# GuyTevet/motion-diffusion-model

Measured on NVIDIA H100. Metric: motions/sec, higher is better.
Workload: dtype fp16 operands / fp32 accumulate (in/out projections hi-lo split)

## Files before the change

motion-diffusion-model_b200/csrc/attention_tc.cuh:

```cuda
#pragma once
#include <cuda_fp16.h>

#include "epilogues.cuh"
#include "ptx.cuh"

namespace b200 {

constexpr int ATC_THREADS = 128;
constexpr int ATC_QROWS = 64;
constexpr int ATC_TILES_PER_CTA = 4;
constexpr int ATC_DH = 128;
constexpr int ATC_MAX_KEYS = 256;

__host__ __device__ constexpr int atc_keys(int S) { return S <= 64 ? 64 : S <= 208 ? 208 : 256; }

struct AttnTcSmem {
  static __host__ __device__ int total(int keys) { return 1024 + 4 * keys * 128; }
};

template <int KEYS, bool WIDE>
__global__ void __launch_bounds__(ATC_THREADS, 2)
attention_tc_kernel(const __grid_constant__ CUtensorMap map_kv, const __half* __restrict__ qkv, __half* __restrict__ out,
                    const int* __restrict__ kvlen, int S, int d, float scale_log2) {
  constexpr int ATOM = KEYS * 128;
  constexpr int NS = KEYS / 2;
  constexpr int NB = KEYS / 16;
  extern __shared__ uint8_t smem_raw[];
  __shared__ uint64_t bar_k, bar_v;
  uint8_t* sK = reinterpret_cast<uint8_t*>((reinterpret_cast<uintptr_t>(smem_raw) + 1023) & ~uintptr_t(1023));
  uint8_t* sV = sK + 2 * ATOM;
  const int warp = threadIdx.x >> 5, lane = threadIdx.x & 31;
  const int h = blockIdx.x, smp = blockIdx.y;
  const int ld = 3 * d;
  const __half* base = qkv + static_cast<size_t>(smp) * S * ld;

  pdl_launch_dependents();
  if (threadIdx.x == 0) {
    tma_prefetch_desc(&map_kv);
    mbar_init(&bar_k, 1);
    mbar_init(&bar_v, 1);
    fence_barrier_init();
  }
  __syncthreads();
  pdl_wait();
  if (threadIdx.x == 0) {
    mbar_expect_tx(&bar_k, 2 * ATOM);
    for (int a = 0; a < 2; ++a) tma_load_3d(sK + a * ATOM, &map_kv, &bar_k, d + h * ATC_DH + 64 * a, 0, smp);
    mbar_expect_tx(&bar_v, 2 * ATOM);
    for (int a = 0; a < 2; ++a) tma_load_3d(sV + a * ATOM, &map_kv, &bar_v, 2 * d + h * ATC_DH + 64 * a, 0, smp);
  }

  const int kvl = min(kvlen[smp], S);
  const int nblk = max(1, (kvl + 15) >> 4);
  const int g = lane >> 2, t = lane & 3;
  const uint64_t desc_k = wgmma_desc_k_sw128(smem_u32(sK));
  const uint64_t desc_v = wgmma_desc_mn_sw128(smem_u32(sV), ATOM);
  const int ntiles = (S + ATC_QROWS - 1) / ATC_QROWS;
  const int ldo = (WIDE ? 2 : 1) * d;

  uint32_t qa[8][4];
  auto load_q = [&](int tile) {
    const int ra = tile * ATC_QROWS + warp * 16 + g, rb = ra + 8;
    const bool va = ra < S, vb = rb < S;
    const uint32_t* pa = reinterpret_cast<const uint32_t*>(base + static_cast<size_t>(va ? ra : 0) * ld + h * ATC_DH);
    const uint32_t* pb = reinterpret_cast<const uint32_t*>(base + static_cast<size_t>(vb ? rb : 0) * ld + h * ATC_DH);
#pragma unroll
    for (int ks = 0; ks < 8; ++ks) {
      qa[ks][0] = va ? pa[8 * ks + t] : 0u;
      qa[ks][1] = vb ? pb[8 * ks + t] : 0u;
      qa[ks][2] = va ? pa[8 * ks + 4 + t] : 0u;
      qa[ks][3] = vb ? pb[8 * ks + 4 + t] : 0u;
    }
  };
  if (static_cast<int>(blockIdx.z) < ntiles) load_q(blockIdx.z);
#pragma unroll 1
  for (int tile = blockIdx.z; tile < ntiles; tile += gridDim.z) {
    const int ra = tile * ATC_QROWS + warp * 16 + g, rb = ra + 8;
    const bool va = ra < S, vb = rb < S;
    float s[NS];
    mbar_wait(&bar_k, 0);
    wgmma_fence();
#pragma unroll
    for (int ks = 0; ks < 8; ++ks)
      WgmmaRA<KEYS, 0>::mma(s, qa[ks], desc_k + (((ks >> 2) * ATOM + (ks & 3) * 32) >> 4), ks != 0);
    wgmma_commit();
    wgmma_wait<0>();
    wgmma_fence_acc(s);
    float mxa = -INFINITY, mxb = -INFINITY;
#pragma unroll
    for (int j = 0; j < NS / 4; ++j)
#pragma unroll
      for (int i = 0; i < 2; ++i) {
        if (8 * j + 2 * t + i < kvl) {
          mxa = fmaxf(mxa, s[4 * j + i]);
          mxb = fmaxf(mxb, s[4 * j + 2 + i]);
        }
      }
#pragma unroll
    for (int o = 1; o < 4; o <<= 1) {
      mxa = fmaxf(mxa, __shfl_xor_sync(0xffffffffu, mxa, o));
      mxb = fmaxf(mxb, __shfl_xor_sync(0xffffffffu, mxb, o));
    }
    const float offa = (mxa == -INFINITY) ? 0.f : mxa * scale_log2;
    const float offb = (mxb == -INFINITY) ? 0.f : mxb * scale_log2;
    auto ex2 = [](float x) {
      float y;
      asm("ex2.approx.ftz.f32 %0, %1;" : "=f"(y) : "f"(x));
      return y;
    };
    uint32_t p[NB][4];
    float suma = 0.f, sumb = 0.f;
#pragma unroll
    for (int j = 0; j < NS / 4; ++j) {
      const int key = 8 * j + 2 * t;
      const float p0 = key < kvl ? ex2(fmaf(s[4 * j], scale_log2, -offa)) : 0.f;
      const float p1 = key + 1 < kvl ? ex2(fmaf(s[4 * j + 1], scale_log2, -offa)) : 0.f;
      const float p2 = key < kvl ? ex2(fmaf(s[4 * j + 2], scale_log2, -offb)) : 0.f;
      const float p3 = key + 1 < kvl ? ex2(fmaf(s[4 * j + 3], scale_log2, -offb)) : 0.f;
      suma += p0 + p1;
      sumb += p2 + p3;
      p[j >> 1][2 * (j & 1)] = pack_half2(p0, p1);
      p[j >> 1][2 * (j & 1) + 1] = pack_half2(p2, p3);
    }
#pragma unroll
    for (int off = 1; off < 4; off <<= 1) {
      suma += __shfl_xor_sync(0xffffffffu, suma, off);
      sumb += __shfl_xor_sync(0xffffffffu, sumb, off);
    }
    const float inva = suma > 0.f ? 1.f / suma : 0.f;
    const float invb = sumb > 0.f ? 1.f / sumb : 0.f;
    float o[64];
    mbar_wait(&bar_v, 0);
    wgmma_fence();
#pragma unroll
    for (int kk = 0; kk < NB; ++kk)
      if (kk < nblk) WgmmaRA<128, 1>::mma(o, p[kk], desc_v + ((kk * 16 * 128) >> 4), kk != 0);
    wgmma_commit();
    if (tile + static_cast<int>(gridDim.z) < ntiles) load_q(tile + gridDim.z);
    wgmma_wait<0>();
    wgmma_fence_acc(o);
    __half* oa = out + (static_cast<size_t>(smp) * S + (va ? ra : 0)) * ldo + h * ATC_DH + 2 * t;
    __half* ob = out + (static_cast<size_t>(smp) * S + (vb ? rb : 0)) * ldo + h * ATC_DH + 2 * t;
#pragma unroll
    for (int j = 0; j < 16; ++j) {
      const float x0 = o[4 * j] * inva, x1 = o[4 * j + 1] * inva, x2 = o[4 * j + 2] * invb, x3 = o[4 * j + 3] * invb;
      const __half2 ha = __floats2half2_rn(x0, x1), hb = __floats2half2_rn(x2, x3);
      if (va) *reinterpret_cast<__half2*>(oa + 8 * j) = ha;
      if (vb) *reinterpret_cast<__half2*>(ob + 8 * j) = hb;
      if (WIDE) {
        const float2 fa = __half22float2(ha), fb = __half22float2(hb);
        if (va) *reinterpret_cast<__half2*>(oa + d + 8 * j) = __floats2half2_rn(x0 - fa.x, x1 - fa.y);
        if (vb) *reinterpret_cast<__half2*>(ob + d + 8 * j) = __floats2half2_rn(x2 - fb.x, x3 - fb.y);
      }
    }
  }
}

}
```

motion-diffusion-model_b200/csrc/engine.cu:

```cuda
#include <cuda.h>
#include <cuda_fp16.h>
#include <cuda_runtime.h>

#include <algorithm>
#include <cmath>
#include <cstdarg>
#include <cstdio>
#include <cstring>
#include <initializer_list>
#include <map>
#include <string>
#include <vector>

#include "../../include/b200mdm.h"
#include "attention_tc.cuh"
#include "epilogues.cuh"
#include "gemm.cuh"
#include "gemm_ln.cuh"
#include "gemm_pingpong.cuh"
#include "chunk_frame.cuh"
#include "joint_guidance.cuh"
#include "compose.cuh"
#include "postprocess.cuh"
#include "kernels.cuh"
// ... 108 lines not shown
  bool operator==(const GraphKey& o) const {
    return mode == o.mode && B == o.B && T == o.T && flags == o.flags && order == o.order && pred == o.pred &&
           imask == o.imask && iweight == o.iweight && imotion == o.imotion && target_g == o.target_g && hs == o.hs &&
           guide == o.guide && chars == o.chars && groups == o.groups && slots == o.slots;
  }
};

struct Workspace {
  int B = 0, T = 0, S = 0, halves = 1, Bp = 0, M = 0, MB = 0;
  int groups = 0;
  float* mp_x0 = nullptr;
  __half *xin16 = nullptr, *hres = nullptr, *qkv16 = nullptr, *att16 = nullptr, *ffn16 = nullptr, *g16 = nullptr;
  float *tok0 = nullptr, *condproj = nullptr, *proj = nullptr, *scale = nullptr, *x_work = nullptr, *eps_buf = nullptr;
  int *kvlen = nullptr, *tvec = nullptr, *action = nullptr;
  CUtensorMap m_xin, m_h16, m_att, m_ffn, m_g16;
  CUtensorMap m_qkv_st, m_ffn_st;
  CUtensorMap m_qkv_kv;
  CUtensorMap m_res_c, m_res_u;
  CUtensorMap m_hres;
  float* pe_bias = nullptr;
  bool cond_set = false;
  int Mt = 0;
  float *encperm = nullptr, *memtok = nullptr, *memproj = nullptr;
  __half *mem16 = nullptr, *qc16 = nullptr, *kvc16 = nullptr;
  unsigned char* memmask = nullptr;
  CUtensorMap m_mem, m_qc_st, m_kvc_st;
  bool prefix_set = false;
  float *cross_mb = nullptr, *cross_u = nullptr, *cross_b = nullptr, *cross_c = nullptr;
  float *tgt_valid = nullptr, *tgt_g = nullptr;
  bool target_set = false;
  int* hs_desc = nullptr;
  bool hs_set = false;
  float* jg_x0 = nullptr;
  float *plms_ring = nullptr, *plms_mid = nullptr, *plms_pred = nullptr;
  int plms_done = -1, plms_order = 0;
  float* dpm_hist = nullptr;
  int dpm_done = -1, dpm_order = 0;
  float *vb_xs = nullptr, *vb_part = nullptr, *vb_terms = nullptr;
  int vb_cap = 0;
  bool vb_live = false;
  SlotState* slots = nullptr;
  cudaGraphExec_t graph_exec = nullptr;
  GraphKey graph_key;
  int graph_kernels = 0;
  unsigned long long last_use = 0;
};

struct b200mdm_engine : Workspace {
  b200mdm_config cfg;
  int d, ff, L, H, JF, Kp_in, N_out_pad;
  int num_sms = 132;
  std::map<std::string, Tensor32> store;
  bool finalized = false;
  __half *w_in3 = nullptr, *w_out3 = nullptr;
  CUtensorMap m_win, m_wout;
  std::vector<LayerW> layers;
  const float *b_in = nullptr, *b_out = nullptr, *pe = nullptr, *w_txt = nullptr, *b_txt = nullptr, *act_emb = nullptr;
  float *temb_hidden = nullptr, *temb_table = nullptr;
  __half* wkv_all = nullptr;
  float* bkv_all = nullptr;
  CUtensorMap m_wkv_all;
  float *tw0 = nullptr, *tb0 = nullptr, *twk = nullptr, *tbk = nullptr, *twsum = nullptr;
  int tG = 0, tdj = 0, tin = 0, tlayers = 0;
  std::vector<float> h_valid;
  float* tab[N_TABLES] = {};
  bool tab_fresh[N_TABLES] = {};
  int* tmap = nullptr;
  int n_steps = 0, sched_cap = 0;
  std::vector<Workspace> pool;
  unsigned long long use_clock = 0;
  std::vector<int> h_kv, h_action;
  std::vector<unsigned char> h_mask;
  std::vector<int> h_hs;
  bool dec = false;
  bool dec_clip = false;
  float* cross_t = nullptr;
  int ctx = 0, s_off = 1;
  int kw = 1;
  const unsigned char* inpaint_mask = nullptr;
  const float* inpaint_weight = nullptr;
  const float* inpaint_motion = nullptr;
  GuideDesc* jg_desc = nullptr;
  GuideDesc h_guide{};
  unsigned guide_terms = 0;
  int* fg_len = nullptr;
  int fg_len_cap = 0;
  std::vector<int> h_fg_len;
  InterPair* ig_pairs = nullptr;
  int ig_pairs_cap = 0;
  std::vector<InterPair> h_ig_pairs;
  PromptWeight* pw_desc = nullptr;
  PromptWeight h_pw{};
  bool pw_set = false;
  unsigned long long noise_seed = 0;
  long long noise_sample_base = 0;
  StepState* state = nullptr;
  cudaStream_t work = nullptr;
  cudaEvent_t ev_in = nullptr, ev_out = nullptr;
  long long launches = 0;
  bool mem_uncond = false;
  float *chain_mem = nullptr, *chain_prefix = nullptr;
  unsigned char* chain_mask = nullptr;
  size_t chain_mem_cap = 0, chain_mask_cap = 0, chain_prefix_cap = 0;
  std::vector<unsigned char> h_chain_mask;
  int chain_n = 0, chain_off = 0, chain_crop = 0, chain_next = -1;
  bool chain_mems = false;
  const float* prefix_src = nullptr;
  bool slot_mode = false;
  int slot_sampler = 0, slot_flags = 0;
  std::vector<unsigned char> slot_busy;
  std::vector<int> slot_left;
  std::vector<int> h_slot_idx;
  struct ChainSlot {
    unsigned long long seed = 0;
    long long g = 0;
    float scale = 0.f;
    int kv = 0, length = 0, off = 0, chunk = 0, n_chunks = 0;
  };
  std::vector<ChainSlot> chain_slot;
  const float *goal_mean = nullptr, *goal_std = nullptr, *goal_src = nullptr;
  double* goal_carry = nullptr;
  float* goal_tgt = nullptr;
  size_t goal_carry_cap = 0, goal_tgt_cap = 0;
  int goal_n = 0;
  bool goal_set = false;
};

template <class T>
static int dalloc(T** p, size_t n, bool zero = false) {
  const cudaError_t err = cudaMalloc(reinterpret_cast<void**>(p), n * sizeof(T));
  if (err != cudaSuccess) {
    cudaGetLastError();
    return fail(B200MDM_ECUDA, "cudaMalloc of %zu bytes failed: %s", n * sizeof(T), cudaGetErrorString(err));
  }
  if (zero) CUDA_TRY(cudaMemset(*p, 0, n * sizeof(T)));
  return B200MDM_OK;
}
template <class T>
static void dfree(T*& p) {
  if (p) cudaFree(p);
  p = nullptr;
}

template <int BN, class Epi>
static int set_gemm_attr() {
  CUDA_TRY(cudaFuncSetAttribute(gemm_f16_wgmma<BN, Epi>, cudaFuncAttributeMaxDynamicSharedMemorySize, GemmSmem<BN, Epi>::TOTAL));
  return B200MDM_OK;
}
template <class Epi>
static int set_pingpong_attr() {
  CUDA_TRY(cudaFuncSetAttribute(gemm_f16_pingpong<Epi>, cudaFuncAttributeMaxDynamicSharedMemorySize, PP_SMEM_BYTES));
  return B200MDM_OK;
}
template <int KEYS>
static int set_attention_attr() {
  CUDA_TRY(cudaFuncSetAttribute(attention_tc_kernel<KEYS, false>, cudaFuncAttributeMaxDynamicSharedMemorySize,
                                AttnTcSmem::total(KEYS)));
  CUDA_TRY(cudaFuncSetAttribute(attention_tc_kernel<KEYS, true>, cudaFuncAttributeMaxDynamicSharedMemorySize,
                                AttnTcSmem::total(KEYS)));
  return B200MDM_OK;
}

enum GuideTerm : unsigned { GT_JOINT = 1, GT_FOOT = 2, GT_SCENE = 4, GT_INTER = 8 };
struct GuideVariant {
  void (*step)(const GuideDesc*, const float*, EpiOutParams);
  void (*test)(GuideDesc, const float*, float*, float*, int, int, int);
  size_t (*smem)(int, int);
  bool clusters;
};
static const GuideVariant GUIDE_VARIANTS[] = {
    {joint_guidance_step_kernel<false, false>, joint_guidance_test_kernel<false, false>, jg_smem_bytes, false},
    {joint_guidance_step_kernel<true, false>, joint_guidance_test_kernel<true, false>, fg_smem_bytes, false},
    {joint_guidance_step_kernel<true, true>, joint_guidance_test_kernel<true, true>, fg_smem_bytes, false},
    {joint_guidance_step_kernel<true, true, true>, joint_guidance_test_kernel<true, true, true>, ig_smem_bytes, true},
};
static int guide_variant(unsigned terms) { return terms ? 31 - __builtin_clz(terms) : -1; }
struct RicDims {
  int J, R;
};
static RicDims ric_dims(int D) {
  const int J = D == 263 ? 22 : 21;
  return {J, 4 + 3 * (J - 1)};
}

static int init_kernel_attrs() {
  static unsigned long long done_mask = 0;
  int dev = 0;
  CUDA_TRY(cudaGetDevice(&dev));
  if (dev < 64 && ((done_mask >> dev) & 1ull)) return B200MDM_OK;
  TRY((set_pingpong_attr<EpiBiasF16<false>>()));
  TRY((set_pingpong_attr<EpiBiasF16<true>>()));
  TRY((set_pingpong_attr<EpiBiasF16Wide<true>>()));
  TRY((set_pingpong_attr<EpiBiasF16Global>()));
  CUDA_TRY(cudaFuncSetAttribute(gemm_resid_ln_cluster, cudaFuncAttributeMaxDynamicSharedMemorySize, GemmLnSmem::TOTAL));
  TRY((set_gemm_attr<128, EpiEmbed>()));
  TRY((set_gemm_attr<96, EpiOut<OutStep>>()));
  TRY((set_gemm_attr<96, EpiOut<OutStepSlots>>()));
  TRY((set_gemm_attr<96, EpiOut<OutPlms>>()));
  TRY((set_gemm_attr<96, EpiOut<OutReverse>>()));
  TRY((set_gemm_attr<96, EpiOut<OutDpm>>()));
  TRY((set_gemm_attr<96, EpiOut<OutVb>>()));
  TRY((set_attention_attr<64>()));
  TRY((set_attention_attr<208>()));
  TRY((set_attention_attr<256>()));
  CUDA_TRY(cudaFuncSetAttribute(cross_attention_long_kernel, cudaFuncAttributeMaxDynamicSharedMemorySize, XAL_SMEM));
  for (const GuideVariant& v : GUIDE_VARIANTS) {
    const int smem = static_cast<int>(v.smem(JG_MAX_FRAMES, JG_MAX_FEATS));
    CUDA_TRY(cudaFuncSetAttribute(v.step, cudaFuncAttributeMaxDynamicSharedMemorySize, smem));
    CUDA_TRY(cudaFuncSetAttribute(v.test, cudaFuncAttributeMaxDynamicSharedMemorySize, smem));
  }
  if (dev < 64) done_mask |= 1ull << dev;
  return B200MDM_OK;
}

static bool g_pdl_now = false;
static bool pdl_enabled() {
  static int v = -1;
  if (v < 0) {
    const char* e = getenv("B200MDM_PDL");
    v = (e && e[0] == '0') ? 0 : 1;
  }
  return v == 1;
}
struct PdlScope {
  PdlScope() { g_pdl_now = pdl_enabled(); }
  ~PdlScope() { g_pdl_now = false; }
};
template <class... KArgs, class... Args>
static cudaError_t launch_kc(void (*kern)(KArgs...), dim3 grid, dim3 block, size_t smem, cudaStream_t s, int cluster,
                             Args&&... args) {
  cudaLaunchConfig_t cfg;
  memset(&cfg, 0, sizeof(cfg));
  cfg.gridDim = grid;
  cfg.blockDim = block;
  cfg.dynamicSmemBytes = smem;
  cfg.stream = s;
  cudaLaunchAttribute at[2];
  int n = 0;
  if (cluster > 0) {
    at[n].id = cudaLaunchAttributeClusterDimension;
    at[n].val.clusterDim.x = static_cast<unsigned>(cluster);
    at[n].val.clusterDim.y = 1;
    at[n].val.clusterDim.z = 1;
    ++n;
  }
  if (g_pdl_now) {
    at[n].id = cudaLaunchAttributeProgrammaticStreamSerialization;
    at[n].val.programmaticStreamSerializationAllowed = 1;
    ++n;
  }
  cfg.attrs = at;
  cfg.numAttrs = n;
  return cudaLaunchKernelEx(&cfg, kern, static_cast<KArgs>(std::forward<Args>(args))...);
}
template <class... KArgs, class... Args>
static cudaError_t launch_k(void (*kern)(KArgs...), dim3 grid, dim3 block, size_t smem, cudaStream_t s, Args&&... args) {
  return launch_kc(kern, grid, block, smem, s, 0, std::forward<Args>(args)...);
}

template <class Epi, class = void> struct epi_unstaged : std::false_type {};
template <class Epi> struct epi_unstaged<Epi, std::enable_if_t<Epi::UNSTAGED>> : std::true_type {};

static_assert(GemmSmem<128, EpiEmbed>::STAGES == 2, "shared-memory budget: 2 operand stages for the embedding GEMM");
static_assert(GemmSmem<96, EpiOut<OutStep>>::STAGES == 5, "shared-memory budget: 5 operand stages for the output GEMM");
template <int BN, class Epi>
static int launch_gemm(const CUtensorMap& a, const CUtensorMap& b, int M, int N, int K, const typename Epi::Params& p,
                       cudaStream_t s, int num_sms) {
  const int tiles = ((M + GEMM_BLOCK_M - 1) / GEMM_BLOCK_M) * ((N + BN - 1) / BN);
  const int grid = tiles < num_sms ? tiles : num_sms;
  CUDA_TRY(launch_k(gemm_f16_wgmma<BN, Epi>, dim3(grid), dim3(GEMM_THREADS), GemmSmem<BN, Epi>::TOTAL, s, a, b, M, N, K, p));
  return B200MDM_OK;
}
template <class Epi>
static int launch_gemm_pp(const CUtensorMap& a, const CUtensorMap& b, const CUtensorMap& c, int M, int N, int K,
                          const typename Epi::Params& p, cudaStream_t s, int num_sms) {
  if (!epi_unstaged<Epi>::value && N * 4 > GEMM_BIAS_BYTES)
    return fail(B200MDM_ENOTIMPL, "GEMM epilogue vectors are staged for N <= %d", GEMM_BIAS_BYTES / 4);
  const int tiles = ((M + GEMM_BLOCK_M - 1) / GEMM_BLOCK_M) * ((N + PP_BLOCK_N - 1) / PP_BLOCK_N);
  const int grid = tiles < num_sms ? tiles : num_sms;
  CUDA_TRY(launch_k(gemm_f16_pingpong<Epi>, dim3(grid), dim3(GEMM_THREADS), PP_SMEM_BYTES, s, a, b, c, M, N, K, p));
  return B200MDM_OK;
}
template <bool GELU>
static int launch_gemm_bias(const CUtensorMap& a, const CUtensorMap& b, const CUtensorMap& c, int M, int N, int K,
                            const float* bias, cudaStream_t s, int num_sms) {
  typename EpiBiasF16<GELU>::Params p{bias};
  return launch_gemm_pp<EpiBiasF16<GELU>>(a, b, c, M, N, K, p, s, num_sms);
}

static int launch_gemm_resid_ln(const CUtensorMap& a, const CUtensorMap& w256, const CUtensorMap& hres, int M, int K,
                                const float* bias, const float* gamma, const float* beta, cudaStream_t s, int num_sms) {
  const int tiles = (M + GEMM_BLOCK_M - 1) / GEMM_BLOCK_M;
  const int max_clusters = num_sms / 2;
  const int clusters = tiles < max_clusters ? tiles : max_clusters;
  GemmLnParams lp{bias, gamma, beta, 1e-5f};
  CUDA_TRY(launch_k(gemm_resid_ln_cluster, dim3(2 * clusters), dim3(GLN_THREADS), GemmLnSmem::TOTAL, s, a, w256, hres, M, K, lp));
  return B200MDM_OK;
}

static int make_attention_kv_map(CUtensorMap* m, const void* qkv, int n_samples, int S, int ld) {
  return make_map_3d(m, qkv, n_samples, S, ld, ld, atc_keys(S));
}
template <int KEYS>
static cudaError_t launch_attention_keys(const CUtensorMap& map_kv, const __half* qkv, __half* out, const int* kvlen,
                                         dim3 grid, int S, int d, float scale_log2, cudaStream_t s, bool wide) {
  return launch_k(wide ? attention_tc_kernel<KEYS, true> : attention_tc_kernel<KEYS, false>, grid, dim3(ATC_THREADS),
                  AttnTcSmem::total(KEYS), s, map_kv, qkv, out, kvlen, S, d, scale_log2);
}
static int launch_attention_tc(const CUtensorMap& map_kv, const __half* qkv, __half* out, const int* kvlen, int n_samples,
                               int S, int d, int H, cudaStream_t s, bool wide = false) {
  if (d != H * ATC_DH) return fail(B200MDM_ENOTIMPL, "attention: head_dim must be 128");
  if (S > ATC_MAX_KEYS) return fail(B200MDM_ENOTIMPL, "attention: at most %d tokens per sample", ATC_MAX_KEYS);
  const float scale_log2 = 1.4426950408889634f / sqrtf(static_cast<float>(ATC_DH));
  const int tiles = (S + ATC_QROWS - 1) / ATC_QROWS;
  const dim3 grid(H, n_samples, (tiles + ATC_TILES_PER_CTA - 1) / ATC_TILES_PER_CTA);
  const int keys = atc_keys(S);
  if (keys == 64) CUDA_TRY(launch_attention_keys<64>(map_kv, qkv, out, kvlen, grid, S, d, scale_log2, s, wide));
  else if (keys == 208) CUDA_TRY(launch_attention_keys<208>(map_kv, qkv, out, kvlen, grid, S, d, scale_log2, s, wide));
  else CUDA_TRY(launch_attention_keys<256>(map_kv, qkv, out, kvlen, grid, S, d, scale_log2, s, wide));
  return B200MDM_OK;
}
static int launch_cross_attention(const __half* q16, const __half* kv, const unsigned char* mask, __half* out, int n_samples,
                                  int S, int Mt, int d, int H, int ld_kv, cudaStream_t s) {
  const float sl2 = 1.4426950408889634f / sqrtf(128.0f);
  const dim3 cg(H, n_samples), cb(128);
  if (Mt <= 16)
    CUDA_TRY(launch_k(cross_attention_kernel<2>, cg, cb, 0, s, q16, kv, mask, out, S, Mt, d, ld_kv, sl2));
  else if (Mt <= 32)
    CUDA_TRY(launch_k(cross_attention_kernel<4>, cg, cb, 0, s, q16, kv, mask, out, S, Mt, d, ld_kv, sl2));
  else if (Mt <= 64)
    CUDA_TRY(launch_k(cross_attention_kernel<8>, cg, cb, 0, s, q16, kv, mask, out, S, Mt, d, ld_kv, sl2));
  else
    CUDA_TRY(launch_k(cross_attention_long_kernel, dim3(H, n_samples, (S + XAL_ROWS - 1) / XAL_ROWS), cb, XAL_SMEM, s, q16, kv,
                      mask, out, S, Mt, d, ld_kv, sl2));
  return B200MDM_OK;
}
static int launch_row_bias_ln(__half* hres, const float* c, const float* gamma, const float* beta, int M, int S, cudaStream_t s) {
  CUDA_TRY(launch_k(row_bias_ln_kernel, dim3((M + RBLN_ROWS_PER_CTA - 1) / RBLN_ROWS_PER_CTA), dim3(32 * RBLN_ROWS_PER_CTA), 0, s,
                    hres, c, gamma, beta, M, S, 1e-5f));
  return B200MDM_OK;
}
static int philox_blocks(int B, long long n) {
  const long long quads = (n + 3) / 4 * B;
  return static_cast<int>(quads / 256 + 1 < 1184 ? quads / 256 + 1 : 1184);
}
static int launch_philox(float* out, int B, long long n, unsigned long long seed, long long sample_base, uint32_t step_id,
                         const StepState* state, cudaStream_t s) {
  CUDA_TRY(launch_k(philox_normal_kernel, dim3(philox_blocks(B, n)), dim3(256), 0, s, out, B, n, seed, sample_base, step_id,
                    state));
  return B200MDM_OK;
}
static int launch_pack_input(const float* x, __half* xin16, int B, int JF, int cols, int S, int Kp, int row_off, cudaStream_t s) {
  CUDA_TRY(launch_k(pack_input_kernel, dim3((cols + 31) / 32, (JF + 31) / 32, B), dim3(32, 8), 0, s, x, xin16, B, JF, cols, S,
                    Kp, 3 * Kp, row_off));
  return B200MDM_OK;
}
static int launch_embed_gemm(const CUtensorMap& m_xin, const CUtensorMap& m_win, const CUtensorMap& m_res_c,
                             const CUtensorMap& m_res_u, const float* pe_bias, int MB, int S, int d, int Kp, int halves,
                             cudaStream_t s, int num_sms) {
  EpiEmbed::Params p;
  p.res_c = m_res_c; p.res_u = m_res_u;
  p.pe_bias = pe_bias;
  p.S = S; p.d = d; p.halves = halves;
  return launch_gemm<128, EpiEmbed>(m_xin, m_win, MB, d, 3 * Kp, p, s, num_sms);
}
static int launch_vb_xt(float* x_t, const float* x_start, const float* noise, const float* sched_vb, const StepState* state,
                        size_t n, cudaStream_t s) {
  const int blocks = static_cast<int>(n / 256 + 1 < 1184 ? n / 256 + 1 : 1184);
  CUDA_TRY(launch_k(vb_xt_kernel, dim3(blocks), dim3(256), 0, s, x_t, x_start, noise, sched_vb, state, n));
  return B200MDM_OK;
}
static int launch_vb_reduce(float* terms, int ld_terms, const float* part, int B, int T, int JF, const StepState* state,
                            cudaStream_t s) {
  CUDA_TRY(launch_k(vb_reduce_kernel, dim3(B, VB_TERMS), dim3(VB_REDUCE_THREADS), 0, s, terms, ld_terms, part, B,
                    T * ((JF + 31) / 32), static_cast<float>(JF) * static_cast<float>(T), state));
  return B200MDM_OK;
}
static int launch_blend_split(const __half* hres, __half* g16, const float* scale, int B, int S, int T, int s_off, int d,
                              int halves, const int* hs, cudaStream_t s) {
  CUDA_TRY(launch_k(blend_split_kernel, dim3((B * T + 7) / 8), dim3(256), 0, s, hres, g16, scale, B, S, T, s_off, d, halves, hs));
  return B200MDM_OK;
}

static int handshake_desc(int h, int B, int T, const int64_t* lengths, const uint8_t* motion_start, std::vector<int>* desc) {
  desc->clear();
  if (h < 0) return fail(B200MDM_EINVAL, "handshake size %d < 0", h);
  if (B <= 0 || T <= 0) return fail(B200MDM_EINVAL, "bad batch / nframes");
  if (motion_start && !motion_start[0]) return fail(B200MDM_EINVAL, "window 0 must begin a motion (motion_start[0])");
  if (h == 0) return B200MDM_OK;
  std::vector<int> d(1 + 2 * static_cast<size_t>(B), 0);
  d[HS_H] = h;
  bool any = false;
  for (int b = 0; b < B; ++b) {
    const long long n = lengths ? lengths[b] : T;
    if (n < 0 || n > T) return fail(B200MDM_EINVAL, "window %d: length %lld outside [0, %d]", b, n, T);
    d[HS_LEN(b)] = static_cast<int>(n);
    d[HS_CHAIN(b)] = (b > 0 && !(motion_start && motion_start[b])) ? 1 : 0;
    any = any || d[HS_CHAIN(b)];
  }
  for (int b = 0; b < B; ++b) {
    const bool prev = d[HS_CHAIN(b)] != 0, next = b + 1 < B && d[HS_CHAIN(b + 1)] != 0;
    const int n = d[HS_LEN(b)];
    if ((prev || next) && n < h) return fail(B200MDM_EINVAL, "chained window %d has %d frames < handshake size %d", b, n, h);
    if (prev && next && n < 2 * h)
      return fail(B200MDM_EINVAL, "window %d has %d frames < 2 x handshake size %d: its two handshakes would overlap", b, n, h);
  }
  if (any) desc->swap(d);
  return B200MDM_OK;
}
#ifdef B200_TRACE
static int debug_skip_mask() {
  static int v = -1;
  if (v < 0) {
    const char* e = getenv("B200MDM_DEBUG_SKIP");
    v = e ? atoi(e) : 0;
  }
  return v;
}
#define B200_SKIP(bit) (debug_skip_mask() & (bit))
#else
#define B200_SKIP(bit) (0)
#endif
extern "C" const char* b200mdm_last_error(void) { return g_err; }
extern "C" int b200mdm_version(void) { return 1; }

extern "C" int b200mdm_create(const b200mdm_config* cfg, b200mdm_engine** out) {
  if (!cfg || !out) return fail(B200MDM_EINVAL, "null argument");
  if (cfg->arch != B200MDM_ARCH_TRANS_ENC && cfg->arch != B200MDM_ARCH_TRANS_DEC)
    return fail(B200MDM_ENOTIMPL, "arch %d: trans_enc and trans_dec are implemented", cfg->arch);
  if (cfg->arch == B200MDM_ARCH_TRANS_DEC && (cfg->cond_mode != B200MDM_COND_TEXT || cfg->context_len < 0))
    return fail(B200MDM_ENOTIMPL, "trans_dec needs text-token conditioning (BERT) and context_len >= 0");
  if (cfg->emb_trans_dec < 0 || cfg->emb_trans_dec > 1 || cfg->dec_memory < B200MDM_DEC_MEMORY_TOKENS ||
      cfg->dec_memory > B200MDM_DEC_MEMORY_CLIP)
    return fail(B200MDM_EINVAL, "emb_trans_dec must be 0 or 1 and dec_memory 0 (tokens) or 1 (CLIP) (got %d / %d)",
                cfg->emb_trans_dec, cfg->dec_memory);
  if (cfg->arch == B200MDM_ARCH_TRANS_ENC && (cfg->emb_trans_dec || cfg->dec_memory))
    return fail(B200MDM_EINVAL, "emb_trans_dec and dec_memory are trans_dec fields");
  if (cfg->arch == B200MDM_ARCH_TRANS_DEC && (cfg->dec_memory == B200MDM_DEC_MEMORY_CLIP) != (cfg->emb_trans_dec == 1))
    return fail(B200MDM_ENOTIMPL, "trans_dec implements the BERT token memory without the timestep token (DiP) and the CLIP "
                "memory with it (emb_trans_dec); got dec_memory %d, emb_trans_dec %d", cfg->dec_memory, cfg->emb_trans_dec);
  if (cfg->dec_memory == B200MDM_DEC_MEMORY_CLIP && cfg->context_len != 0)
    return fail(B200MDM_ENOTIMPL, "trans_dec with a CLIP memory has no prefix completion (context_len %d)", cfg->context_len);
  if (cfg->latent_dim != 512 || cfg->num_heads != 4 || cfg->ff_size % 64 || cfg->ff_size <= 0)
    return fail(B200MDM_ENOTIMPL, "kernels are specialised for latent_dim 512 / 4 heads (got %d / %d)", cfg->latent_dim,
                cfg->num_heads);
  if (cfg->num_layers <= 0 || cfg->njoints <= 0 || cfg->nfeats <= 0 || cfg->pos_embed_max_len <= 0 || cfg->temb_rows <= 0)
    return fail(B200MDM_EINVAL, "bad config");
  if (cfg->target_encoder < B200MDM_TARGET_NONE || cfg->target_encoder > B200MDM_TARGET_SPLIT)
    return fail(B200MDM_EINVAL, "target_encoder %d: 0 none, 1 single, 2 multi, 3 split", cfg->target_encoder);
  if (cfg->target_encoder != B200MDM_TARGET_NONE) {
    if (cfg->target_joints <= 0 || cfg->target_joints > 64 || cfg->target_enc_layers < 0 || cfg->target_enc_layers > 16)
      return fail(B200MDM_EINVAL, "target encoder: 1..64 joints and 0..16 layers (got %d / %d)", cfg->target_joints,
                  cfg->target_enc_layers);
    if (cfg->target_encoder == B200MDM_TARGET_SPLIT && cfg->latent_dim % cfg->target_joints)
      return fail(B200MDM_EINVAL, "split target encoder: latent_dim %% target_joints != 0 (model/mdm.py:427)");
  }
  int dev = 0;
  CUDA_TRY(cudaGetDevice(&dev));
  cudaDeviceProp prop;
  CUDA_TRY(cudaGetDeviceProperties(&prop, dev));
  if (prop.major != 9 || prop.minor != 0) return fail(B200MDM_ECUDA, "sm_90a device required (found sm_%d%d)", prop.major, prop.minor);
  TRY(init_kernel_attrs());
  TRY(resolve_driver());
  b200mdm_engine* e = new b200mdm_engine();
  e->cfg = *cfg;
  e->d = cfg->latent_dim;
  e->ff = cfg->ff_size;
  e->L = cfg->num_layers;
  e->H = cfg->num_heads;
  e->JF = cfg->njoints * cfg->nfeats;
  e->Kp_in = (e->JF + 7) & ~7;
  e->N_out_pad = ((e->JF + 95) / 96) * 96;
  e->num_sms = prop.multiProcessorCount;
// ... 2780 lines not shown
```

Measured before the change: 429.8.

## Make self-attention kernel persistent over (sample, head) items with K/V prefetch

Turns the attention kernel into a persistent kernel whose grid is sized to resident CTAs, computed from occupancy queries at init. Each CTA loops over (sample, head) items and handles all query tiles itself. The TMA loads of K and V for the next item are issued once the current item's last tile has consumed them, and each 64-column half gets its own mbarrier so the QK product can start on the first half early. The aim is to cut K/V reloads and launch/tail overhead and to overlap loads with compute. In exchange it adds __syncthreads calls, per-device static state, and less parallelism per item, since one CTA now walks every tile serially.

```diff
diff --git a/motion-diffusion-model_b200/csrc/attention_tc.cuh b/motion-diffusion-model_b200/csrc/attention_tc.cuh
--- a/motion-diffusion-model_b200/csrc/attention_tc.cuh
+++ b/motion-diffusion-model_b200/csrc/attention_tc.cuh
@@ -8,7 +8,6 @@
 
 constexpr int ATC_THREADS = 128;
 constexpr int ATC_QROWS = 64;
-constexpr int ATC_TILES_PER_CTA = 4;
 constexpr int ATC_DH = 128;
 constexpr int ATC_MAX_KEYS = 256;
 
@@ -21,37 +20,42 @@
 template <int KEYS, bool WIDE>
 __global__ void __launch_bounds__(ATC_THREADS, 2)
 attention_tc_kernel(const __grid_constant__ CUtensorMap map_kv, const __half* __restrict__ qkv, __half* __restrict__ out,
-                    const int* __restrict__ kvlen, int S, int d, float scale_log2) {
+                    const int* __restrict__ kvlen, int n_samples, int S, int d, float scale_log2) {
   constexpr int ATOM = KEYS * 128;
   constexpr int NS = KEYS / 2;
   constexpr int NB = KEYS / 16;
   extern __shared__ uint8_t smem_raw[];
-  __shared__ uint64_t bar_k, bar_v;
+  __shared__ uint64_t bar_k[2], bar_v[2];
   uint8_t* sK = reinterpret_cast<uint8_t*>((reinterpret_cast<uintptr_t>(smem_raw) + 1023) & ~uintptr_t(1023));
   uint8_t* sV = sK + 2 * ATOM;
   const int warp = threadIdx.x >> 5, lane = threadIdx.x & 31;
-  const int h = blockIdx.x, smp = blockIdx.y;
+  const int H = d / ATC_DH, items = n_samples * H;
   const int ld = 3 * d;
-  const __half* base = qkv + static_cast<size_t>(smp) * S * ld;
+
+  auto load_kv = [&](uint64_t* bar, uint8_t* dst, int col, int item) {
+    const int h = item % H, smp = item / H;
+    for (int a = 0; a < 2; ++a) {
+      mbar_expect_tx(&bar[a], ATOM);
+      tma_load_3d(dst + a * ATOM, &map_kv, &bar[a], col + h * ATC_DH + 64 * a, 0, smp);
+    }
+  };
 
   pdl_launch_dependents();
   if (threadIdx.x == 0) {
     tma_prefetch_desc(&map_kv);
-    mbar_init(&bar_k, 1);
-    mbar_init(&bar_v, 1);
+    for (int a = 0; a < 2; ++a) {
+      mbar_init(&bar_k[a], 1);
+      mbar_init(&bar_v[a], 1);
+    }
     fence_barrier_init();
   }
   __syncthreads();
   pdl_wait();
-  if (threadIdx.x == 0) {
-    mbar_expect_tx(&bar_k, 2 * ATOM);
-    for (int a = 0; a < 2; ++a) tma_load_3d(sK + a * ATOM, &map_kv, &bar_k, d + h * ATC_DH + 64 * a, 0, smp);
-    mbar_expect_tx(&bar_v, 2 * ATOM);
-    for (int a = 0; a < 2; ++a) tma_load_3d(sV + a * ATOM, &map_kv, &bar_v, 2 * d + h * ATC_DH + 64 * a, 0, smp);
+  if (threadIdx.x == 0 && static_cast<int>(blockIdx.x) < items) {
+    load_kv(bar_k, sK, d, blockIdx.x);
+    load_kv(bar_v, sV, 2 * d, blockIdx.x);
   }
 
-  const int kvl = min(kvlen[smp], S);
-  const int nblk = max(1, (kvl + 15) >> 4);
   const int g = lane >> 2, t = lane & 3;
   const uint64_t desc_k = wgmma_desc_k_sw128(smem_u32(sK));
   const uint64_t desc_v = wgmma_desc_mn_sw128(smem_u32(sV), ATOM);
@@ -59,11 +63,12 @@
   const int ldo = (WIDE ? 2 : 1) * d;
 
   uint32_t qa[8][4];
-  auto load_q = [&](int tile) {
+  auto load_q = [&](int item, int tile) {
+    const __half* base = qkv + static_cast<size_t>(item / H) * S * ld + (item % H) * ATC_DH;
     const int ra = tile * ATC_QROWS + warp * 16 + g, rb = ra + 8;
     const bool va = ra < S, vb = rb < S;
-    const uint32_t* pa = reinterpret_cast<const uint32_t*>(base + static_cast<size_t>(va ? ra : 0) * ld + h * ATC_DH);
-    const uint32_t* pb = reinterpret_cast<const uint32_t*>(base + static_cast<size_t>(vb ? rb : 0) * ld + h * ATC_DH);
+    const uint32_t* pa = reinterpret_cast<const uint32_t*>(base + static_cast<size_t>(va ? ra : 0) * ld);
+    const uint32_t* pb = reinterpret_cast<const uint32_t*>(base + static_cast<size_t>(vb ? rb : 0) * ld);
 #pragma unroll
     for (int ks = 0; ks < 8; ++ks) {
       qa[ks][0] = va ? pa[8 * ks + t] : 0u;
@@ -72,85 +77,117 @@
       qa[ks][3] = vb ? pb[8 * ks + 4 + t] : 0u;
     }
   };
-  if (static_cast<int>(blockIdx.z) < ntiles) load_q(blockIdx.z);
+  if (static_cast<int>(blockIdx.x) < items) load_q(blockIdx.x, 0);
+  uint32_t phase = 0;
 #pragma unroll 1
-  for (int tile = blockIdx.z; tile < ntiles; tile += gridDim.z) {
-    const int ra = tile * ATC_QROWS + warp * 16 + g, rb = ra + 8;
-    const bool va = ra < S, vb = rb < S;
-    float s[NS];
-    mbar_wait(&bar_k, 0);
-    wgmma_fence();
+  for (int item = blockIdx.x; item < items; item += gridDim.x, phase ^= 1) {
+    const int h = item % H, smp = item / H;
+    const int next = item + gridDim.x;
+    const int kvl = min(kvlen[smp], S);
+    const int nblk = max(1, (kvl + 15) >> 4);
+#pragma unroll 1
+    for (int tile = 0; tile < ntiles; ++tile) {
+      const bool last = tile + 1 == ntiles;
+      const int ra = tile * ATC_QROWS + warp * 16 + g, rb = ra + 8;
+      const bool va = ra < S, vb = rb < S;
+      const bool live = tile * ATC_QROWS + warp * 16 < S;
+      float s[NS];
+      mbar_wait(&bar_k[0], phase);
+      wgmma_fence();
 #pragma unroll
-    for (int ks = 0; ks < 8; ++ks)
-      WgmmaRA<KEYS, 0>::mma(s, qa[ks], desc_k + (((ks >> 2) * ATOM + (ks & 3) * 32) >> 4), ks != 0);
-    wgmma_commit();
-    wgmma_wait<0>();
-    wgmma_fence_acc(s);
-    float mxa = -INFINITY, mxb = -INFINITY;
+      for (int ks = 0; ks < 4; ++ks) WgmmaRA<KEYS, 0>::mma(s, qa[ks], desc_k + ((ks * 32) >> 4), ks != 0);
+      mbar_wait(&bar_k[1], phase);
 #pragma unroll
-    for (int j = 0; j < NS / 4; ++j)
+      for (int ks = 4; ks < 8; ++ks) WgmmaRA<KEYS, 0>::mma(s, qa[ks], desc_k + ((ATOM + (ks & 3) * 32) >> 4), true);
+      wgmma_commit();
+      wgmma_wait<0>();
+      wgmma_fence_acc(s);
+      if (last && next < items) {
+        __syncthreads();
+        if (threadIdx.x == 0) load_kv(bar_k, sK, d, next);
+      }
+      uint32_t p[NB][4];
+      float inva = 0.f, invb = 0.f;
+      if (live) {
+        float mxa = -INFINITY, mxb = -INFINITY;
 #pragma unroll
-      for (int i = 0; i < 2; ++i) {
-        if (8 * j + 2 * t + i < kvl) {
-          mxa = fmaxf(mxa, s[4 * j + i]);
-          mxb = fmaxf(mxb, s[4 * j + 2 + i]);
+        for (int j = 0; j < NS / 4; ++j)
+#pragma unroll
+          for (int i = 0; i < 2; ++i) {
+            if (8 * j + 2 * t + i < kvl) {
+              mxa = fmaxf(mxa, s[4 * j + i]);
+              mxb = fmaxf(mxb, s[4 * j + 2 + i]);
+            }
+          }
+#pragma unroll
+        for (int o = 1; o < 4; o <<= 1) {
+          mxa = fmaxf(mxa, __shfl_xor_sync(0xffffffffu, mxa, o));
+          mxb = fmaxf(mxb, __shfl_xor_sync(0xffffffffu, mxb, o));
         }
+        const float offa = (mxa == -INFINITY) ? 0.f : mxa * scale_log2;
+        const float offb = (mxb == -INFINITY) ? 0.f : mxb * scale_log2;
+        auto ex2 = [](float x) {
+          float y;
+          asm("ex2.approx.ftz.f32 %0, %1;" : "=f"(y) : "f"(x));
+          return y;
+        };
+        float suma = 0.f, sumb = 0.f;
+#pragma unroll
+        for (int j = 0; j < NS / 4; ++j) {
+          const int key = 8 * j + 2 * t;
+          const float p0 = key < kvl ? ex2(fmaf(s[4 * j], scale_log2, -offa)) : 0.f;
+          const float p1 = key + 1 < kvl ? ex2(fmaf(s[4 * j + 1], scale_log2, -offa)) : 0.f;
+          const float p2 = key < kvl ? ex2(fmaf(s[4 * j + 2], scale_log2, -offb)) : 0.f;
+          const float p3 = key + 1 < kvl ? ex2(fmaf(s[4 * j + 3], scale_log2, -offb)) : 0.f;
+          suma += p0 + p1;
+          sumb += p2 + p3;
+          p[j >> 1][2 * (j & 1)] = pack_half2(p0, p1);
+          p[j >> 1][2 * (j & 1) + 1] = pack_half2(p2, p3);
+        }
+#pragma unroll
+        for (int off = 1; off < 4; off <<= 1) {
+          suma += __shfl_xor_sync(0xffffffffu, suma, off);
+          sumb += __shfl_xor_sync(0xffffffffu, sumb, off);
+        }
+        inva = suma > 0.f ? 1.f / suma : 0.f;
+        invb = sumb > 0.f ? 1.f / sumb : 0.f;
+      } else {
+#pragma unroll
+        for (int kk = 0; kk < NB; ++kk)
+#pragma unroll
+          for (int i = 0; i < 4; ++i) p[kk][i] = 0u;
       }
+      float o[64];
+      mbar_wait(&bar_v[0], phase);
+      mbar_wait(&bar_v[1], phase);
+      wgmma_fence();
 #pragma unroll
-    for (int o = 1; o < 4; o <<= 1) {
-      mxa = fmaxf(mxa, __shfl_xor_sync(0xffffffffu, mxa, o));
-      mxb = fmaxf(mxb, __shfl_xor_sync(0xffffffffu, mxb, o));
-    }
-    const float offa = (mxa == -INFINITY) ? 0.f : mxa * scale_log2;
-    const float offb = (mxb == -INFINITY) ? 0.f : mxb * scale_log2;
-    auto ex2 = [](float x) {
-      float y;
-      asm("ex2.approx.ftz.f32 %0, %1;" : "=f"(y) : "f"(x));
-      return y;
-    };
-    uint32_t p[NB][4];
-    float suma = 0.f, sumb = 0.f;
+      for (int kk = 0; kk < NB; ++kk)
+        if (kk < nblk) WgmmaRA<128, 1>::mma(o, p[kk], desc_v + ((kk * 16 * 128) >> 4), kk != 0);
+      wgmma_commit();
+      if (!last) load_q(item, tile + 1);
+      else if (next < items) load_q(next, 0);
+      wgmma_wait<0>();
+      wgmma_fence_acc(o);
+      if (last && next < items) {
+        __syncthreads();
+        if (threadIdx.x == 0) load_kv(bar_v, sV, 2 * d, next);
+      }
+      if (live) {
+        __half* oa = out + (static_cast<size_t>(smp) * S + (va ? ra : 0)) * ldo + h * ATC_DH + 2 * t;
+        __half* ob = out + (static_cast<size_t>(smp) * S + (vb ? rb : 0)) * ldo + h * ATC_DH + 2 * t;
 #pragma unroll
-    for (int j = 0; j < NS / 4; ++j) {
-      const int key = 8 * j + 2 * t;
-      const float p0 = key < kvl ? ex2(fmaf(s[4 * j], scale_log2, -offa)) : 0.f;
-      const float p1 = key + 1 < kvl ? ex2(fmaf(s[4 * j + 1], scale_log2, -offa)) : 0.f;
-      const float p2 = key < kvl ? ex2(fmaf(s[4 * j + 2], scale_log2, -offb)) : 0.f;
-      const float p3 = key + 1 < kvl ? ex2(fmaf(s[4 * j + 3], scale_log2, -offb)) : 0.f;
-      suma += p0 + p1;
-      sumb += p2 + p3;
-      p[j >> 1][2 * (j & 1)] = pack_half2(p0, p1);
-      p[j >> 1][2 * (j & 1) + 1] = pack_half2(p2, p3);
-    }
-#pragma unroll
-    for (int off = 1; off < 4; off <<= 1) {
-      suma += __shfl_xor_sync(0xffffffffu, suma, off);
-      sumb += __shfl_xor_sync(0xffffffffu, sumb, off);
-    }
-    const float inva = suma > 0.f ? 1.f / suma : 0.f;
-    const float invb = sumb > 0.f ? 1.f / sumb : 0.f;
-    float o[64];
-    mbar_wait(&bar_v, 0);
-    wgmma_fence();
-#pragma unroll
-    for (int kk = 0; kk < NB; ++kk)
-      if (kk < nblk) WgmmaRA<128, 1>::mma(o, p[kk], desc_v + ((kk * 16 * 128) >> 4), kk != 0);
-    wgmma_commit();
-    if (tile + static_cast<int>(gridDim.z) < ntiles) load_q(tile + gridDim.z);
-    wgmma_wait<0>();
-    wgmma_fence_acc(o);
-    __half* oa = out + (static_cast<size_t>(smp) * S + (va ? ra : 0)) * ldo + h * ATC_DH + 2 * t;
-    __half* ob = out + (static_cast<size_t>(smp) * S + (vb ? rb : 0)) * ldo + h * ATC_DH + 2 * t;
-#pragma unroll
-    for (int j = 0; j < 16; ++j) {
-      const float x0 = o[4 * j] * inva, x1 = o[4 * j + 1] * inva, x2 = o[4 * j + 2] * invb, x3 = o[4 * j + 3] * invb;
-      const __half2 ha = __floats2half2_rn(x0, x1), hb = __floats2half2_rn(x2, x3);
-      if (va) *reinterpret_cast<__half2*>(oa + 8 * j) = ha;
-      if (vb) *reinterpret_cast<__half2*>(ob + 8 * j) = hb;
-      if (WIDE) {
-        const float2 fa = __half22float2(ha), fb = __half22float2(hb);
-        if (va) *reinterpret_cast<__half2*>(oa + d + 8 * j) = __floats2half2_rn(x0 - fa.x, x1 - fa.y);
-        if (vb) *reinterpret_cast<__half2*>(ob + d + 8 * j) = __floats2half2_rn(x2 - fb.x, x3 - fb.y);
+        for (int j = 0; j < 16; ++j) {
+          const float x0 = o[4 * j] * inva, x1 = o[4 * j + 1] * inva, x2 = o[4 * j + 2] * invb, x3 = o[4 * j + 3] * invb;
+          const __half2 ha = __floats2half2_rn(x0, x1), hb = __floats2half2_rn(x2, x3);
+          if (va) *reinterpret_cast<__half2*>(oa + 8 * j) = ha;
+          if (vb) *reinterpret_cast<__half2*>(ob + 8 * j) = hb;
+          if (WIDE) {
+            const float2 fa = __half22float2(ha), fb = __half22float2(hb);
+            if (va) *reinterpret_cast<__half2*>(oa + d + 8 * j) = __floats2half2_rn(x0 - fa.x, x1 - fa.y);
+            if (vb) *reinterpret_cast<__half2*>(ob + d + 8 * j) = __floats2half2_rn(x2 - fb.x, x3 - fb.y);
+          }
+        }
       }
     }
   }
diff --git a/motion-diffusion-model_b200/csrc/engine.cu b/motion-diffusion-model_b200/csrc/engine.cu
--- a/motion-diffusion-model_b200/csrc/engine.cu
+++ b/motion-diffusion-model_b200/csrc/engine.cu
@@ -284,12 +284,21 @@
   CUDA_TRY(cudaFuncSetAttribute(gemm_f16_pingpong<Epi>, cudaFuncAttributeMaxDynamicSharedMemorySize, PP_SMEM_BYTES));
   return B200MDM_OK;
 }
+constexpr int ATC_MAX_DEVICES = 64;
+static int atc_resident[ATC_MAX_DEVICES][3][2];
+static int atc_keys_index(int keys) { return keys == 64 ? 0 : keys == 208 ? 1 : 2; }
 template <int KEYS>
-static int set_attention_attr() {
-  CUDA_TRY(cudaFuncSetAttribute(attention_tc_kernel<KEYS, false>, cudaFuncAttributeMaxDynamicSharedMemorySize,
-                                AttnTcSmem::total(KEYS)));
-  CUDA_TRY(cudaFuncSetAttribute(attention_tc_kernel<KEYS, true>, cudaFuncAttributeMaxDynamicSharedMemorySize,
-                                AttnTcSmem::total(KEYS)));
+static int set_attention_attr(int dev) {
+  int sms = 0;
+  CUDA_TRY(cudaDeviceGetAttribute(&sms, cudaDevAttrMultiProcessorCount, dev));
+  for (int wide = 0; wide < 2; ++wide) {
+    auto kern = wide ? attention_tc_kernel<KEYS, true> : attention_tc_kernel<KEYS, false>;
+    CUDA_TRY(cudaFuncSetAttribute(kern, cudaFuncAttributeMaxDynamicSharedMemorySize, AttnTcSmem::total(KEYS)));
+    int per_sm = 0;
+    CUDA_TRY(cudaOccupancyMaxActiveBlocksPerMultiprocessor(&per_sm, kern, ATC_THREADS, AttnTcSmem::total(KEYS)));
+    if (per_sm < 1) return fail(B200MDM_ECUDA, "attention: the %d-key kernel does not fit on an SM", KEYS);
+    if (dev < ATC_MAX_DEVICES) atc_resident[dev][atc_keys_index(KEYS)][wide] = per_sm * sms;
+  }
   return B200MDM_OK;
 }
 
@@ -332,9 +341,9 @@
   TRY((set_gemm_attr<96, EpiOut<OutReverse>>()));
   TRY((set_gemm_attr<96, EpiOut<OutDpm>>()));
   TRY((set_gemm_attr<96, EpiOut<OutVb>>()));
-  TRY((set_attention_attr<64>()));
-  TRY((set_attention_attr<208>()));
-  TRY((set_attention_attr<256>()));
+  TRY((set_attention_attr<64>(dev)));
+  TRY((set_attention_attr<208>(dev)));
+  TRY((set_attention_attr<256>(dev)));
   CUDA_TRY(cudaFuncSetAttribute(cross_attention_long_kernel, cudaFuncAttributeMaxDynamicSharedMemorySize, XAL_SMEM));
   for (const GuideVariant& v : GUIDE_VARIANTS) {
     const int smem = static_cast<int>(v.smem(JG_MAX_FRAMES, JG_MAX_FEATS));
@@ -434,23 +443,27 @@
   return make_map_3d(m, qkv, n_samples, S, ld, ld, atc_keys(S));
 }
 template <int KEYS>
-static cudaError_t launch_attention_keys(const CUtensorMap& map_kv, const __half* qkv, __half* out, const int* kvlen,
-                                         dim3 grid, int S, int d, float scale_log2, cudaStream_t s, bool wide) {
-  return launch_k(wide ? attention_tc_kernel<KEYS, true> : attention_tc_kernel<KEYS, false>, grid, dim3(ATC_THREADS),
-                  AttnTcSmem::total(KEYS), s, map_kv, qkv, out, kvlen, S, d, scale_log2);
+static int launch_attention_keys(const CUtensorMap& map_kv, const __half* qkv, __half* out, const int* kvlen,
+                                 int n_samples, int S, int d, float scale_log2, cudaStream_t s, bool wide) {
+  int dev = 0;
+  CUDA_TRY(cudaGetDevice(&dev));
+  const int resident = dev < ATC_MAX_DEVICES ? atc_resident[dev][atc_keys_index(KEYS)][wide] : 0;
+  if (resident < 1) return fail(B200MDM_ESTATE, "attention: kernel attributes of device %d not initialised", dev);
+  const int items = n_samples * (d / ATC_DH);
+  const dim3 grid(KEYS == 64 || items < resident ? items : resident);
+  CUDA_TRY(launch_k(wide ? attention_tc_kernel<KEYS, true> : attention_tc_kernel<KEYS, false>, grid, dim3(ATC_THREADS),
+                    AttnTcSmem::total(KEYS), s, map_kv, qkv, out, kvlen, n_samples, S, d, scale_log2));
+  return B200MDM_OK;
 }
 static int launch_attention_tc(const CUtensorMap& map_kv, const __half* qkv, __half* out, const int* kvlen, int n_samples,
                                int S, int d, int H, cudaStream_t s, bool wide = false) {
   if (d != H * ATC_DH) return fail(B200MDM_ENOTIMPL, "attention: head_dim must be 128");
   if (S > ATC_MAX_KEYS) return fail(B200MDM_ENOTIMPL, "attention: at most %d tokens per sample", ATC_MAX_KEYS);
   const float scale_log2 = 1.4426950408889634f / sqrtf(static_cast<float>(ATC_DH));
-  const int tiles = (S + ATC_QROWS - 1) / ATC_QROWS;
-  const dim3 grid(H, n_samples, (tiles + ATC_TILES_PER_CTA - 1) / ATC_TILES_PER_CTA);
   const int keys = atc_keys(S);
-  if (keys == 64) CUDA_TRY(launch_attention_keys<64>(map_kv, qkv, out, kvlen, grid, S, d, scale_log2, s, wide));
-  else if (keys == 208) CUDA_TRY(launch_attention_keys<208>(map_kv, qkv, out, kvlen, grid, S, d, scale_log2, s, wide));
-  else CUDA_TRY(launch_attention_keys<256>(map_kv, qkv, out, kvlen, grid, S, d, scale_log2, s, wide));
-  return B200MDM_OK;
+  if (keys == 64) return launch_attention_keys<64>(map_kv, qkv, out, kvlen, n_samples, S, d, scale_log2, s, wide);
+  if (keys == 208) return launch_attention_keys<208>(map_kv, qkv, out, kvlen, n_samples, S, d, scale_log2, s, wide);
+  return launch_attention_keys<256>(map_kv, qkv, out, kvlen, n_samples, S, d, scale_log2, s, wide);
 }
 static int launch_cross_attention(const __half* q16, const __half* kv, const unsigned char* mask, __half* out, int n_samples,
                                   int S, int Mt, int d, int H, int ld_kv, cudaStream_t s) {
```

Result: no change. 426.4, median of 6 (-0.8%).
